# vita-epfl/collaborative-gan-sampling

Hardware: AMD Instinct MI355X
Metric: refined samples/sec @ 20 refinement steps (higher is better)
Workload: dtype f32; 1 GPU; dcgan64 collaborative refinement (propose + K-step refine + render), batch 1024/GPU, K=20, momentum rate 0.1, refine at feature [8, 8, 256], random-init weights, z~U(-1,1) seed 2019+rank; global_batch=1024, refine_steps=20, parallelism=single GPU, hipgraph=True, batches_in_flight=2, fused_per_launch=1, sync_bn=False, contraction=f32

## Files before the change

collaborative-gan-sampling_amd/csrc/api.hip:

```cpp
#include <stdarg.h>
#include <stdio.h>

#include "cgs_internal.h"

static thread_local char g_err[512] = "";
static thread_local const char* g_last_kernel = "";

static thread_local double g_last_flops = 0.0;
static thread_local int g_last_tail[2] = {0, 0};
void cgs_note_tail(int tiles, int split) { g_last_tail[0] = tiles; g_last_tail[1] = split; }
static thread_local int g_contraction = CGS_CONTRACTION_F32;
int cgs_contraction_mode() { return g_contraction; }

void cgs_note_kernel(const char* name) { g_last_kernel = name; }
void cgs_note_flops(double f) { g_last_flops = f; }
void cgs_add_flops(double f) { g_last_flops += f; }

int cgs_set_error(int code, const char* fmt, ...) {
    va_list ap;
    va_start(ap, fmt);
    vsnprintf(g_err, sizeof(g_err), fmt, ap);
    va_end(ap);
    return code;
}

extern "C" {

int cgs_version(void) { return 117; }
const char* cgs_last_error(void) { return g_err; }
const char* cgs_last_kernel(void) { return g_last_kernel; }
double cgs_last_executed_flops(void) { return g_last_flops; }
int cgs_last_tail_tiles(void) { return g_last_tail[0]; }
int cgs_last_tail_split(void) { return g_last_tail[1]; }
int cgs_set_contraction(int mode) {
    if (mode < CGS_CONTRACTION_F32 || mode > CGS_CONTRACTION_BX6_ALL) return cgs_set_error(CGS_EINVAL, "set_contraction: mode %d", mode);
    g_contraction = mode;
    return CGS_OK;
}
int cgs_get_contraction(void) { return g_contraction; }

}

struct ConvCall { CgsLayer L; bool dirT, deconv, bwd; };

static ConvCall conv_call_of(int op, int H, int W, int Cin, int Ho, int Wo, int Cout, int kh, int kw, int sh, int sw) {
    ConvCall c;
    c.deconv = (op == CGS_DECONV_FWD || op == CGS_DECONV_BWD_DATA);
    c.bwd = (op == CGS_CONV_BWD_DATA || op == CGS_DECONV_BWD_DATA);
    c.dirT = (op == CGS_CONV_BWD_DATA || op == CGS_DECONV_FWD);
    CgsLayer& L = c.L;
    L.kh = kh; L.kw = kw; L.sh = sh; L.sw = sw;
    if (!c.deconv) { L.Hb = H; L.Wb = W; L.Cb = Cin; L.Hs = cgs_ceil_div(H, sh > 0 ? sh : 1); L.Ws = cgs_ceil_div(W, sw > 0 ? sw : 1); L.Cs = Cout; }
    else { L.Hs = H; L.Ws = W; L.Cs = Cin; L.Hb = Ho; L.Wb = Wo; L.Cb = Cout; }
    return c;
}

static int check_layer(const CgsLayer& L, const char* who) {
    if (L.kh <= 0 || L.kw <= 0 || L.sh <= 0 || L.sw <= 0 || L.Hb <= 0 || L.Wb <= 0 || L.Cb <= 0 || L.Cs <= 0)
        return cgs_set_error(CGS_EINVAL, "%s: non-positive dimension", who);
    if (L.Hs != cgs_ceil_div(L.Hb, L.sh) || L.Ws != cgs_ceil_div(L.Wb, L.sw))
        return cgs_set_error(CGS_EINVAL, "%s: 'SAME' geometry mismatch: big %dx%d stride %dx%d needs small %dx%d, got %dx%d", who,
// ... 523 lines not shown
```

collaborative-gan-sampling_amd/csrc/bn.hip:

```cpp
#include "cgs_internal.h"

#define BN_MAX_BLOCKS CGS_BN_MAX_BLOCKS

struct BnGeom {
    int G;
    int rows_per_block;
};

static BnGeom bn_geom(int M, int C) {
    BnGeom g;
    int rpb = cgs_ceil_div(M, BN_MAX_BLOCKS);
    if (rpb < 16) rpb = 16;
    g.rows_per_block = rpb;
    g.G = cgs_ceil_div(M, rpb);
    (void)C;
    return g;
}

__device__ __forceinline__ float4 zero4() { return make_float4(0.f, 0.f, 0.f, 0.f); }

__device__ __forceinline__ void bn_affine4(const float* __restrict__ mean, const float* __restrict__ invstd, const float* __restrict__ gamma,
                                           const float* __restrict__ beta, int c, float4& mu, float4& inv, float4& sc, float4& sh) {
    mu = *(const float4*)(mean + c); inv = *(const float4*)(invstd + c);
    const float4 g = *(const float4*)(gamma + c), b = *(const float4*)(beta + c);
// ... 649 lines not shown
        return cgs_set_error(CGS_EWORKSPACE, "groupnorm fwd from partials: workspace %zu < %zu", ws_bytes, (size_t)groups * 4 * C * sizeof(float));
    return norm_fwd_from_partials("groupnorm_lrelu_fwd_from_partials", x, part, groups, rows_per_seg, nseg, seg_stride, gamma, beta, eps, leak, y, mean, invstd,
                                  M_group, C, (float*)ws , nullptr, (hipStream_t)stream);
}

int cgs_norm_lrelu_bwd_from_partials(const float* dy, const float* x, const float* part, int groups, int rows_per_seg, int nseg, int seg_stride,
                                     const float* gamma, const float* beta, const float* mean, const float* invstd, float leak, float* dx,
                                     int M_group, int C, void* ws, size_t ws_bytes, void* stream) {
    const char* who = "norm_lrelu_bwd_from_partials";
    if (groups <= 0 || groups > 65535 || M_group <= 0 || C <= 0 || (C & 3) || rows_per_seg <= 0 || nseg <= 0 || seg_stride < 0 || !part || !dy || !x || !dx)
        return cgs_set_error(CGS_EINVAL, "norm bwd from partials: groups=%d M=%d C=%d rows=%d x %d", groups, M_group, C, rows_per_seg, nseg);
    const bool sliced = groups == 1 && nseg == 1 && rows_per_seg >= 1024 && !((uintptr_t)ws & 7);
    const size_t need = (size_t)groups * 2 * C * sizeof(float) + (sliced ? (size_t)BNF_SLICES * 2 * C * sizeof(double) : 0);
    if (!ws || ws_bytes < need) return cgs_set_error(CGS_EWORKSPACE, "norm bwd from partials: workspace %zu < %zu", ws_bytes, need);
    hipStream_t s = (hipStream_t)stream;
    if (const int rpb = norm_fa_rows_per_block(groups, rows_per_seg, nseg, M_group, C)) {
        hipLaunchKernelGGL(norm_fa_kernel<true>, dim3(cgs_ceil_div(C, 64), cgs_ceil_div(M_group, rpb), groups), dim3(256), 0, s, x, dy, part, rows_per_seg, nseg,
                           seg_stride, gamma, beta, 0.f, leak, dx, (float*)mean, (float*)invstd, M_group, C, rpb);
        return norm_launched(who, "norm_fa_bwd");
    }
    float* stat2 = (float*)ws;
    if (sliced) {
        double* slices = (double*)ws;
        stat2 = (float*)(slices + (size_t)BNF_SLICES * 2 * C);
        hipLaunchKernelGGL(bn_slice_sums_kernel, dim3(cgs_ceil_div(C, BNF_CH), BNF_SLICES), dim3(256), 0, s, part, rows_per_seg, C, slices);
        hipLaunchKernelGGL(bn_finalize2_slices_kernel, dim3(cgs_ceil_div(C, 64)), dim3(64), 0, s, slices, BNF_SLICES, (double)M_group, C, stat2);
    } else {
        hipLaunchKernelGGL(bn_finalize_kernel<1>, dim3(cgs_ceil_div(C, BNF_CH), groups), dim3(256), 0, s, part, rows_per_seg, M_group, C, nullptr, nullptr, 0.f,
                           stat2, nullptr, nullptr, nseg, seg_stride);
    }
    launch_apply_bwd(dy, x, mean, invstd, gamma, beta, stat2, leak, dx, groups, M_group, C, s);
    return norm_launched(who, sliced ? "norm_sliced_bwd" : "norm_finalize_bwd");
}
```

collaborative-gan-sampling_amd/engine.py:

```python
import gc

import numpy as np
import torch

from . import kernels as K
from . import lib as L
from .nets import ARCHS, _same_out, g_input_shape, layer_ks


class _Stage:
    out = None
    bwd_epi = (L.EPI_NONE, None, None)
    pre_folded = False
    bwd_nstat = None
    bstat = None

    def fwd(self, x):
        raise NotImplementedError

    def bwd(self, dy):
        raise NotImplementedError


class _View(_Stage):
# ... 416 lines not shown
            continue
        if isinstance(below, _BnTrainLrelu) and below.sync is None:
            gamma, beta, gimg = below.gamma, below.beta, B // below.groups
        elif isinstance(below, _InstNormAct):
            gamma, beta, gimg = below.scale, below.offset, 1
        else:
            continue
        C = below.out.shape[-1]
        if isinstance(above, _Conv):
            H, W, Cin = above.dx.shape[1:]
            kh, kw, _, Cout = above.w.shape
            lay = K.conv_stat_layout(L.CONV_BWD_DATA, B, H, W, Cin, 0, 0, Cout, kh, kw, above.s, above.s, gimg)
        else:
            lay = K.conv_stat_layout(L.DECONV_BWD_DATA, *above.call_dims(), above.s, above.s, gimg)
        if lay is None:
            continue
        part = torch.empty((lay[0], 2, C), dtype=torch.float32, device=below.out.device)
        below.bstat = above.bwd_nstat = K.NormBwdStats(None, below.mean, below.invstd, gamma, beta, below.leak, gimg, part, lay)
    if stages and isinstance(stages[-1], _Residual):
        link_norm_backward_stats(stages[-1].inner, B)


class Tape:

    def __init__(self, layers, in_shape, P, scope, B, k, stride, bn_training, dev):
        self.folds = []
        self.stages, self.out_shape = compile_layers(layers, in_shape, P, scope, B, k, stride, bn_training, dev, self.folds)

    def forward(self, x):
        for st in self.stages:
            x = st.fwd(x)
        return x

    def backward(self, dy, update=None):
        for st in reversed(self.stages[1:]):
            dy = st.bwd(dy)
        return self.stages[0].bwd(dy) if update is None else self.stages[0].bwd(dy, update=update)


def _entry(fn):
    import functools

    @functools.wraps(fn)
    def wrapped(self, *a, **kw):
        prev = K.set_contraction(self.contraction)
        try:
            return fn(self, *a, **kw)
        finally:
            if prev != self.contraction:
                K.set_contraction(prev)
    return wrapped


class RefineEngine:

    def __init__(self, arch, params, batch_size, device=None, use_graph=False, sync_bn=None, bn_groups=1, contraction="f32"):
        self.A = ARCHS[arch] if isinstance(arch, str) else arch
        if contraction not in L.CONTRACTIONS:
            raise L.CgsError(f"contraction {contraction!r}: expected one of {sorted(L.CONTRACTIONS)}")
        self.contraction = contraction
        self.dev = torch.device(device if device is not None else "cuda:0")
        if self.dev.type != "cuda":
            raise L.CgsError("RefineEngine needs a GPU device (there is no CPU path)")
        L.load()
        prev_mode = K.set_contraction(self.contraction)
        try:
            self._build(params, batch_size, use_graph, sync_bn, bn_groups)
        finally:
# ... 33 lines not shown
                for below, st in zip([None] + stages[:-1], stages):
                    if isinstance(st, _BnTrainLrelu):
                        st.set_groups(self.bn_groups, below if isinstance(below, _Conv) else None)
                    if isinstance(st, _Residual):
                        walk_g(st.inner)
            walk_g(self.d.stages); walk_g(self.g_tail.stages)
        self.sync_bn = None
        if sync_bn is not None and sync_bn is not False:
            if use_graph:
                raise L.CgsError("sync_bn runs eagerly: the all-reduce between the two halves of a bn pass is not captured")
            self.sync_bn = BnSync(None if sync_bn is True else sync_bn)

            def walk(stages):
                for st in stages:
                    if isinstance(st, _BnTrainLrelu):
                        st.sync = self.sync_bn
                    if isinstance(st, _Residual):
                        walk(st.inner)
            walk(self.d.stages); walk(self.g_tail.stages)

        def drop_partials(stages):
            for below, st in zip([None] + stages[:-1], stages):
                if isinstance(st, _BnTrainLrelu) and st.sync is not None:
                    st.part = None
                    if isinstance(below, _Conv):
                        below.part = None
                if isinstance(st, _Residual):
                    drop_partials(st.inner)
        drop_partials(self.d.stages); drop_partials(self.g_tail.stages)
        link_norm_backward_stats(self.g_tail.stages + self.d.stages, B)
        first = self.g_tail.stages[0]
        self.update_form = first.update_form() if isinstance(first, (_Conv, _Deconv)) else None
        self.fused_update = self.update_form is not None and self.update_form[0] != "tail"

    def _sync_weights(self):
        if self._ws_epoch != K.WS.epoch:
            self._resync()

    def _resync(self):
        K.set_contraction(self.contraction)
        epoch = K.WS.epoch
        with torch.cuda.device(self.dev):
            for tape in (self.g_head, self.g_tail, self.d):
                for a, c, gamma, beta, mm, mv in tape.folds:
                    K.bn_fold(gamma, beta, mm, mv, out=(a, c))
            if self._gstream is not None and self._graphs:
                cur = torch.cuda.current_stream(self.dev)
                self._gstream.wait_stream(cur)
                with torch.cuda.stream(self._gstream):
                    self.forward_logits(self.theta, self.logit)
                    self.backward_to_feature()
                cur.wait_stream(self._gstream)
        self._ws_epoch = epoch

    @_entry
    def input_to_feature(self, z):
        self._sync_weights()
        return self.g_head.forward(z)

    @_entry
    def feature_to_data(self, feat):
        self._sync_weights()
        return self.g_tail.forward(feat)

    @_entry
    def discriminator(self, x):
# ... 18 lines not shown
            i -= 1
        st = stages[i] if i >= 0 else None
        active = (isinstance(st, (_Conv, _Linear)) and st.epi != L.EPI_NONE) or (isinstance(st, (_BnTrainLrelu, _InstNormAct)) and st.leak != 1.0) \
            or isinstance(st, _Unary)
        if not active:
            raise L.CgsError("score_with_features: no nonlinearity in front of the discriminator's logit layer")
        return st

    def feature_width(self):
        return int(self._feature_stage().out.shape[-1])

    @_entry
    def score_with_features(self, images, out=None, feat_out=None):
        self._sync_weights()
        st = self._feature_stage()
        sig = K.sigmoid_rowmean(self.d.forward(images), out=out)
        act = st.out
        if act.dim() == 2:
            if feat_out is None:
                return sig, act
            feat_out.copy_(act)
            return sig, feat_out
        if feat_out is None:
            if getattr(self, "_feat", None) is None:
                self._feat = torch.empty((act.shape[0], act.shape[-1]), dtype=torch.float32, device=self.dev)
            feat_out = self._feat
        return sig, K.spatial_mean(act, out=feat_out)

    def forward_logits(self, theta, logit_out, loss="bce", ladam=None, first=False):
        x = self.g_tail.forward(theta)
        head = self.d.stages[-1]
        plain = loss == "bce" and ladam is None
        if isinstance(head, _Linear) and head.w.shape[1] == 1 and head.epi == L.EPI_NONE:
            for st in self.d.stages[:-1]:
                x = st.fwd(x)
            head.x_in = x
            if plain:
                return K.linear_out1_bce(x, head.w, head.b, head.out, self.dlogits, logit_out)
            return K.linear_out1_seed(x, head.w, head.b, head.out, self.dlogits, logit_out, loss, ladam, first)
        logits = self.d.forward(x)
        if plain:
            K.bce_ones_grad_rowmean(logits, self.dlogits, logit_out)
        else:
            K.refine_loss_seed(logits, loss, self.dlogits, logit_out, ladam, first)
        return logits

    def backward_to_feature(self, update=None):
        return self.g_tail.backward(self.d.backward(self.dlogits), update=update)

    @_entry
    def compute_forward_logits_and_grad(self, feature, loss="bce"):
        if loss not in ("bce", "lsq", "linear"):
            raise L.CgsError(f"loss {loss!r}: the engine differentiates 'bce', 'lsq' and 'linear'")
        self._sync_weights()
        self.forward_logits(feature, self.logit, loss)
        return self.logit, self.backward_to_feature()

    def _program(self, steps, rate, alpha, probabilistic, vmin, vmax, loss="bce", ladam=None):
        th = self.theta
        render = self.g_tail.stages[-1].out
        self.forward_logits(th, self.logit, loss, ladam, True)
        self.default_logit.copy_(self.logit)
        self.best_logit.copy_(self.logit)
        self.best_theta.copy_(th)
        self.images.copy_(render)
        self.best_step.fill_(1.0)
        self.tickets.zero_()
        forced = self.forced if probabilistic else None
        fused = self.fused_update and self.update_form is not None and ladam is None and not (vmin and vmax)
        for i in range(steps):
            if fused:
                self.backward_to_feature(update=K.FusedUpdate(th, self.mom, rate, alpha, first=(i == 0)))
                self.forward_logits(th, self.logit, loss, ladam, False)
                K.refine_select2(render, self.images, th, self.best_theta, self.logit, forced, i, self.best_logit, self.best_step, self.tickets)
                continue
            g = self.backward_to_feature()
            if ladam is None:
                K.refine_update(th, self.mom, g, rate, alpha, first=(i == 0), vmin=vmin, vmax=vmax)
            else:
                K.refine_update_ladam(th, self.mom, self.mean_square, g, ladam.gain, rate, first=(i == 0), vmin=vmin, vmax=vmax)
            self.forward_logits(th, self.logit, loss, ladam, False)
            K.refine_select2(render, self.images, th, self.best_theta, self.logit, forced, i, self.best_logit, self.best_step, self.tickets)

    @_entry
    def refine(self, feature0, steps, rate, method="momentum", mode="deterministic", indices=None,
               vmin=None, vmax=None, loss="bce", real_sigmoid_mean=None):
        ladam = None
        if method == "momentum":
            alpha = 0.9
        elif method == "sgd":
            alpha = 0.0
        elif method == "ladam":
            if real_sigmoid_mean is None:
                raise L.CgsError("ladam needs a loss argument the map-space refiner never passes "
                                 "(sampling/collaborator.py:66 vs policy.py:48-51); use momentum or sgd, or pass real_sigmoid_mean")
            alpha = None
        else:
            raise NotImplementedError(method)
        if loss not in ("bce", "lsq", "linear"):
            raise L.CgsError(f"loss {loss!r}: the engine differentiates 'bce', 'lsq' and 'linear'")
        if mode not in ("deterministic", "probabilistic"):
            raise NotImplementedError(mode)
        prob = mode == "probabilistic"
        if prob:
            if indices is None:
                raise L.CgsError("probabilistic mode needs the step indices (np.random.randint(K+1, size=B))")
            self.forced.copy_(torch.as_tensor(np.asarray(indices), dtype=torch.int32))
        if tuple(feature0.shape) != tuple(self.theta.shape):
            raise L.CgsError(f"feature batch {tuple(feature0.shape)} != engine shape {tuple(self.theta.shape)}")
        self._sync_weights()
        with torch.cuda.device(self.dev):
            self.theta.copy_(feature0)
            if method == "ladam":
                if self._ladam is None:
                    self._ladam = K.LadamState(self.B, self.dev)
                    self.mean_square = torch.empty_like(self.mom)
                ladam = self._ladam
                ladam.set_real(real_sigmoid_mean)
            key = (steps, float(rate), alpha, prob, vmin, vmax, loss, method, bool(self.fused_update))
            if not self.use_graph:
                self._program(steps, rate, alpha, prob, vmin, vmax, loss, ladam)
            else:
                g = self._graphs.get(key)
                if g is None:
                    if self._gstream is None:
                        self._gstream = torch.cuda.Stream(self.dev)
                    cur = torch.cuda.current_stream(self.dev)
                    self._gstream.wait_stream(cur)
                    with torch.cuda.stream(self._gstream):
                        self._program(steps, rate, alpha, prob, vmin, vmax, loss, ladam)
                        self.theta.copy_(feature0)
                    torch.cuda.synchronize(self.dev)
                    gc_was_on = gc.isenabled()
                    gc.disable()
                    try:
                        g = torch.cuda.CUDAGraph()
                        with torch.cuda.graph(g, stream=self._gstream, capture_error_mode="thread_local"):
                            self._program(steps, rate, alpha, prob, vmin, vmax, loss, ladam)
                    except L.CgsError:
                        raise
                    except Exception as ex:
                        raise L.GraphCaptureError(f"{type(ex).__name__}: {str(ex)[:300]}") from ex
                    finally:
                        if gc_was_on:
                            gc.enable()
                    cur.wait_stream(self._gstream)
                    self._graphs[key] = g
                g.replay()
        return self.images, self.default_logit, self.best_logit, self.best_step, self.best_theta

    @_entry
    def refresh_weights(self):
# ... 7 lines not shown
```

collaborative-gan-sampling_amd/kernels.py:

```python
import math
import operator
import weakref

import torch

from . import lib as L

LEAK = 0.2
BN_EPS = 1e-5


def _chk(t, name):
    if not (isinstance(t, torch.Tensor) and t.is_cuda and t.dtype == torch.float32 and t.is_contiguous()):
        raise L.CgsError(f"{name}: expected a contiguous fp32 tensor on the GPU, got "
                         f"{type(t).__name__} {getattr(t, 'dtype', None)} {getattr(t, 'device', None)}")
    return t


def _ptr(t):
    return None if t is None else t.data_ptr()


def _stream():
    return torch.cuda.current_stream().cuda_stream
# ... 687 lines not shown
        self.loss_avg = torch.empty(B, dtype=torch.float32, device=device)
        self.gain = torch.empty(B, dtype=torch.float32, device=device)

    def set_real(self, value):
        if isinstance(value, torch.Tensor):
            self.s_real.copy_(value.reshape(1))
        else:
            self.s_real.fill_(float(value))

    def arg(self, first):
        import ctypes
        return ctypes.byref(L.LadamSeed(_ptr(self.s_real), _ptr(self.loss_avg), _ptr(self.gain), 1 if first else 0))


def refine_loss_seed(logits, kind, dlogits=None, logit_mean=None, ladam=None, first=False):
    _chk(logits, "logits")
    B = logits.shape[0]
    dl = dlogits if dlogits is not None else torch.empty_like(logits)
    lm = logit_mean if logit_mean is not None else torch.empty(B, dtype=torch.float32, device=logits.device)
    L.call("cgs_refine_loss_seed", _ptr(logits), _loss_kind(kind, ("bce", "lsq", "linear")), _ptr(dl), _ptr(lm), B, logits.numel() // B,
           None if ladam is None else ladam.arg(first), _stream())
    return dl, lm


def linear_out1_seed(x, w, bias, logits, dlogits, logit_mean, kind, ladam=None, first=False):
    _chk(x, "x"); _chk(w, "w")
    B, K = x.shape
    pr = _Prof(2.0 * B * K, "", _nb(x, w, logits), op="linear_out1_fwd") if PROFILE is not None else None
    L.call("cgs_linear_out1_seed", _ptr(x), _ptr(w), _ptr(bias), _ptr(logits), _ptr(dlogits), _ptr(logit_mean), B, K,
           _loss_kind(kind, ("bce", "lsq", "linear")), None if ladam is None else ladam.arg(first), _stream())
    if pr is not None:
        pr.done()
    return logits


def ladam_gain(loss, loss_avg, gain, first):
    for t, name in ((loss, "loss"), (loss_avg, "loss_avg"), (gain, "gain")):
        _chk(t, name)
    B = loss.numel()
    if loss_avg.numel() != B or gain.numel() != B:
        raise L.CgsError("ladam_gain: loss, loss_avg and gain must have one size")
    L.call("cgs_ladam_gain", _ptr(loss), _ptr(loss_avg), _ptr(gain), 1 if first else 0, B, _stream())
    return gain


def refine_update_ladam(theta, m, v, g, gain, rate, first, vmin=None, vmax=None):
    for t, name in ((theta, "theta"), (m, "m"), (v, "v"), (g, "g"), (gain, "gain")):
        _chk(t, name)
    B = theta.shape[0]
    if m.numel() != theta.numel() or v.numel() != theta.numel() or g.numel() != theta.numel() or gain.numel() < B:
        raise L.CgsError("refine_update_ladam: theta, m, v and g must have one size, gain at least B elements")
    use_clip = 1 if (vmin and vmax) else 0
    pr = _Prof(0.0, "", _nb(theta, theta, m, v, g) + (0.0 if first else _nb(m, v)), op="refine_update_ladam") if PROFILE is not None else None
    L.call("cgs_refine_update_ladam", _ptr(theta), _ptr(m), _ptr(v), _ptr(g), _ptr(gain), float(rate), 1 if first else 0, use_clip,
           float(vmin or 0.0), float(vmax or 0.0), B, theta.numel() // B, _stream())
    if pr is not None:
        pr.done()


def refine_select_rows(src, logit, forced, step_index, dst, best_logit):
    B = src.shape[0]
    L.call("cgs_refine_select_rows", _ptr(src), _ptr(logit), _ptr(forced), step_index, _ptr(dst), _ptr(best_logit),
           B, src.numel() // B, _stream())


_wgrad_ws = {}
# ... 513 lines not shown
```

collaborative-gan-sampling_amd/lib.py:

```python
import ctypes as C
import os

_HERE = os.path.dirname(os.path.abspath(__file__))
LIB_PATH = os.environ.get("CGS_LIB") or os.path.join(_HERE, "libcgs_hip.so")

OK, EINVAL, EWORKSPACE, ELAUNCH = 0, -1, -2, -3
EPI_NONE, EPI_LRELU, EPI_AFFINE_RELU, EPI_TANH = 0, 1, 2, 3
EPI_RELU_BWD_AFFINE, EPI_LRELU_BWD, EPI_TANH_BWD = 4, 5, 6
CONV_FWD, CONV_BWD_DATA, DECONV_FWD, DECONV_BWD_DATA = 0, 1, 2, 3
FAMILY_IGEMM, FAMILY_QUAD, FAMILY_SMALLN_T, FAMILY_SMALLN_F, FAMILY_PATCH, FAMILY_TAPS, FAMILY_DOT, FAMILY_IGEMM_BX6 = 0, 1, 2, 3, 4, 5, 6, 7
CONTRACTION_F32, CONTRACTION_BX6, CONTRACTION_BX6_ALL = 0, 1, 2
CONTRACTIONS = {"f32": CONTRACTION_F32, "bx6": CONTRACTION_BX6, "bx6_all": CONTRACTION_BX6_ALL}
LOSS_BCE, LOSS_LSQ, LOSS_LINEAR, LOSS_HINGE = 0, 1, 2, 3
LOSSES = {"bce": LOSS_BCE, "lsq": LOSS_LSQ, "linear": LOSS_LINEAR, "hinge": LOSS_HINGE}


class LadamSeed(C.Structure):
    _fields_ = [("s_real", C.c_void_p), ("loss_avg", C.c_void_p), ("gain", C.c_void_p), ("first", C.c_int)]


_p, _i, _f, _z = C.c_void_p, C.c_int, C.c_float, C.c_size_t
_ll = C.c_longlong

SIGNATURES = {
# ... 10 lines not shown
    "cgs_conv_ws_bytes_for": (_z, [_i] * 10),
    "cgs_conv_family": (_i, [_i] * 13 + [_z]),
    "cgs_conv2d_nhwc_fwd": (_i, [_p] * 4 + [_i] * 9 + [_i, _p, _p, _p, _z, _i, _p]),
    "cgs_conv_stat_partials": (_i, [_i] * 9 + [_z]),
    "cgs_conv2d_nhwc_fwd_stats": (_i, [_p] * 4 + [_i] * 9 + [_p, _z, _i, _p, _z, _p]),
    "cgs_conv_stat_layout": (_i, [_i] * 13 + [_z, _p, _p, _p]),
    "cgs_deconv2d_nhwc_fwd_stats": (_i, [_p] * 4 + [_i] * 11 + [_p, _z, _i, _p, _z, _p]),
    "cgs_conv2d_nhwc_bwd_data_nstats": (_i, [_p] * 3 + [_i] * 9 + [_p] * 5 + [_f, _i, _p, _z, _i, _p, _z, _p]),
    "cgs_deconv2d_nhwc_bwd_data_nstats": (_i, [_p] * 3 + [_i] * 11 + [_p] * 5 + [_f, _i, _p, _z, _i, _p, _z, _p]),
    "cgs_norm_lrelu_bwd_from_partials": (_i, [_p] * 3 + [_i] * 4 + [_p] * 4 + [_f, _p, _i, _i, _p, _z, _p]),
    "cgs_groupnorm_lrelu_fwd_from_partials": (_i, [_p, _p, _i, _i, _i, _i, _p, _p, _f, _f, _p, _p, _p, _i, _i, _p, _z, _p]),
    "cgs_bn_train_lrelu_fwd_from_partials": (_i, [_p, _p, _i, _p, _p, _f, _f, _p, _p, _p, _i, _i, _p, _z, _p]),
    "cgs_conv2d_nhwc_bwd_data": (_i, [_p] * 3 + [_i] * 9 + [_i, _p, _p, _p, _z, _i, _p]),
    "cgs_deconv2d_nhwc_fwd": (_i, [_p] * 4 + [_i] * 11 + [_i, _p, _p, _p, _z, _i, _p]),
    "cgs_deconv2d_nhwc_bwd_data": (_i, [_p] * 3 + [_i] * 11 + [_i, _p, _p, _p, _z, _i, _p]),
    "cgs_conv_update_form": (_i, [_i] * 12 + [_z, _p]),
    "cgs_conv2d_nhwc_bwd_data_update": (_i, [_p] * 4 + [_i] * 9 + [_f, _f, _i, _p, _z, _i, _p]),
    "cgs_deconv2d_nhwc_bwd_data_update": (_i, [_p] * 4 + [_i] * 11 + [_f, _f, _i, _p, _z, _i, _p]),
    "cgs_conv_signs_ok": (_i, [_i] * 13 + [_z]),
    "cgs_deconv2d_nhwc_fwd_signs": (_i, [_p] * 4 + [_i] * 11 + [_i, _p, _p, _p, _p, _z, _i, _p]),
    "cgs_deconv2d_nhwc_bwd_data_signs": (_i, [_p] * 3 + [_i] * 11 + [_i, _p, _p, _p, _z, _i, _p]),
    "cgs_linear_fwd": (_i, [_p] * 4 + [_i] * 4 + [_p, _z, _i, _p]),
    "cgs_linear_bwd_data": (_i, [_p] * 3 + [_i] * 3 + [_p, _z, _i, _p]),
    "cgs_bn_ws_bytes": (_z, [_i, _i]),
    "cgs_bn_train_lrelu_fwd": (_i, [_p, _p, _p, _f, _f, _p, _p, _p, _i, _i, _p, _z, _p]),
    "cgs_bn_train_lrelu_bwd_data": (_i, [_p] * 6 + [_f, _p, _i, _i, _p, _z, _p]),
    "cgs_bn_sync_fwd_sums": (_i, [_p, _p, _i, _i, _p, _z, _p]),
    "cgs_bn_sync_fwd_apply": (_i, [_p, _p, _p, _f, _f, _p, _ll, _p, _p, _p, _i, _i, _p, _z, _p]),
    "cgs_bn_sync_bwd_sums": (_i, [_p] * 6 + [_f, _p, _i, _i, _p, _z, _p]),
    "cgs_bn_sync_bwd_apply": (_i, [_p] * 6 + [_f, _p, _ll, _p, _i, _i, _p, _z, _p]),
    "cgs_instnorm_ws_bytes": (_z, [_i, _i, _i]),
    "cgs_instnorm_lrelu_fwd": (_i, [_p, _p, _p, _f, _f, _p, _p, _p, _i, _i, _i, _p, _z, _p]),
    "cgs_instnorm_lrelu_bwd_data": (_i, [_p] * 6 + [_f, _p, _i, _i, _i, _p, _z, _p]),
    "cgs_add": (_i, [_p, _p, _p, _z, _p]),
    "cgs_bn_fold": (_i, [_p] * 4 + [_f, _p, _p, _i, _p]),
    "cgs_affine_relu_fwd": (_i, [_p] * 4 + [_i, _i, _p]),
    "cgs_affine_relu_bwd": (_i, [_p] * 4 + [_i, _i, _p]),
    "cgs_affine_fwd": (_i, [_p] * 4 + [_i, _i, _p]),
    "cgs_affine_bwd": (_i, [_p] * 3 + [_i, _i, _p]),
    "cgs_lrelu_fwd": (_i, [_p, _f, _p, _z, _p]),
    "cgs_lrelu_bwd": (_i, [_p, _p, _f, _p, _z, _p]),
    "cgs_tanh_fwd": (_i, [_p, _p, _z, _p]),
    "cgs_tanh_bwd": (_i, [_p, _p, _p, _z, _p]),
    "cgs_bce_ones_grad_rowmean": (_i, [_p, _p, _p, _i, _i, _p]),
    "cgs_bce_ones_fwd": (_i, [_p, _p, _z, _p]),
    "cgs_bce_ones_bwd": (_i, [_p, _p, _p, _z, _p]),
    "cgs_sigmoid_rowmean": (_i, [_p, _p, _i, _i, _p]),
    "cgs_clip": (_i, [_p, _f, _f, _p, _z, _p]),
    "cgs_refine_update": (_i, [_p, _p, _p, _f, _f, _i, _i, _f, _f, _z, _p]),
    "cgs_refine_select": (_i, [_p, _p, _p, _i, _p, _p, _p, _i, _i, _p]),
    "cgs_refine_select_rows": (_i, [_p, _p, _p, _i, _p, _p, _i, _i, _p]),
    "cgs_refine_select2": (_i, [_p, _p, _i, _p, _p, _i, _p, _p, _i, _p, _p, _p, _i, _p]),
    "cgs_linear_out1_bce": (_i, [_p, _p, _p, _p, _p, _p, _i, _i, _p]),
    "cgs_linear_out1_seed": (_i, [_p, _p, _p, _p, _p, _p, _i, _i, _i, _p, _p]),
    "cgs_refine_loss_seed": (_i, [_p, _i, _p, _p, _i, _i, _p, _p]),
    "cgs_refine_update_ladam": (_i, [_p, _p, _p, _p, _p, _f, _i, _i, _f, _f, _i, _i, _p]),
    "cgs_ladam_gain": (_i, [_p, _p, _p, _i, _i, _p]),
    "cgs_gan_logits_grad": (_i, [_p, _i, _f, _f, _p, _p, _i, _p]),
    "cgs_gan_loss": (_i, [_p, _i, _f, _p, _p, _z, _p]),
    "cgs_mlp2d_sigmoid_saliency": (_i, [_p, _p, _i, _i, _p, _p, _p, _i, _f, _p]),
    "cgs_refine2d": (_i, [_p, _p, _i, _i, _p, _f, _f, _i, _f, _i, _p, _p, _p, _i, _p]),
    "cgs_refine2d_devbase": (_i, [_p, _p, _i, _i, _p, _p, _f, _i, _f, _i, _p, _p, _p, _i, _p]),
    "cgs_mlp2d_train_ws_bytes": (_z, [_i, _i]),
    "cgs_mlp2d_d_step": (_i, [_p, _p, _i, _i, _p, _i, _p, _i, _f, _p, _p, _p, _p, _z, _p]),
    "cgs_mlp2d_wide_train_ws_bytes": (_z, [_i, _i, _i]),
    "cgs_mlp2d_wide_d_step": (_i, [_p, _p, _i, _i, _p, _i, _p, _i, _f, _p, _p, _p, _p, _z, _p]),
# ... 145 lines not shown
```

include/cgs_hip.h:

```cpp
#ifndef CGS_HIP_H
#define CGS_HIP_H

#include <stddef.h>
#include <stdint.h>

#ifdef __cplusplus
extern "C" {
#endif

#define CGS_OK 0
#define CGS_EINVAL (-1)
#define CGS_EWORKSPACE (-2)
#define CGS_ELAUNCH (-3)

#define CGS_EPI_NONE 0
#define CGS_EPI_LRELU 1
#define CGS_EPI_AFFINE_RELU 2
#define CGS_EPI_TANH 3
#define CGS_EPI_RELU_BWD_AFFINE 4
#define CGS_EPI_LRELU_BWD 5
#define CGS_EPI_TANH_BWD 6

#define CGS_CONV_FWD 0
#define CGS_CONV_BWD_DATA 1
// ... 121 lines not shown
int cgs_linear_bwd_data(const float* dy, const float* w, float* dx, int B, int in, int out,
                        void* ws, size_t ws_bytes, int ws_prepacked, void* stream);

size_t cgs_bn_ws_bytes(int M, int C);
int cgs_bn_train_lrelu_fwd(const float* x, const float* gamma, const float* beta, float eps, float leak,
                           float* y, float* mean, float* invstd, int M, int C,
                           void* ws, size_t ws_bytes, void* stream);
int cgs_bn_train_lrelu_fwd_from_partials(const float* x, const float* part, int G, const float* gamma, const float* beta,
                                         float eps, float leak, float* y, float* mean, float* invstd, int M, int C,
                                         void* ws, size_t ws_bytes, void* stream);
int cgs_bn_train_lrelu_bwd_data(const float* dy, const float* x, const float* gamma, const float* beta,
                                const float* mean, const float* invstd, float leak, float* dx, int M, int C,
                                void* ws, size_t ws_bytes, void* stream);

int cgs_bn_sync_fwd_sums(const float* x, double* sums, int M, int C, void* ws, size_t ws_bytes, void* stream);
int cgs_bn_sync_fwd_apply(const float* x, const float* gamma, const float* beta, float eps, float leak, const double* sums,
                          long long M_total, float* y, float* mean, float* invstd, int M, int C,
                          void* ws, size_t ws_bytes, void* stream);
int cgs_bn_sync_bwd_sums(const float* dy, const float* x, const float* gamma, const float* beta, const float* mean,
                         const float* invstd, float leak, double* sums, int M, int C, void* ws, size_t ws_bytes, void* stream);
int cgs_bn_sync_bwd_apply(const float* dy, const float* x, const float* gamma, const float* beta, const float* mean,
                          const float* invstd, float leak, const double* sums, long long M_total, float* dx, int M, int C,
                          void* ws, size_t ws_bytes, void* stream);

size_t cgs_instnorm_ws_bytes(int B, int HW, int C);
int cgs_instnorm_lrelu_fwd(const float* x, const float* scale, const float* offset, float eps, float leak, float* y,
                           float* mean, float* invstd, int B, int HW, int C, void* ws, size_t ws_bytes, void* stream);
int cgs_instnorm_lrelu_bwd_data(const float* dy, const float* x, const float* scale, const float* offset,
                                const float* mean, const float* invstd, float leak, float* dx, int B, int HW, int C,
                                void* ws, size_t ws_bytes, void* stream);
int cgs_groupnorm_lrelu_fwd_from_partials(const float* x, const float* part, int groups, int rows_per_seg, int nseg, int seg_stride,
                                          const float* gamma, const float* beta, float eps, float leak, float* y, float* mean,
                                          float* invstd, int M_group, int C, void* ws, size_t ws_bytes, void* stream);
int cgs_add(const float* a, const float* b, float* out, size_t n, void* stream);

int cgs_bn_fold(const float* gamma, const float* beta, const float* moving_mean, const float* moving_var,
                float eps, float* a, float* b, int C, void* stream);
int cgs_affine_relu_fwd(const float* x, const float* a, const float* b, float* y, int M, int C, void* stream);
int cgs_affine_relu_bwd(const float* dy, const float* y, const float* a, float* dx, int M, int C, void* stream);
int cgs_affine_fwd(const float* x, const float* a, const float* b, float* y, int M, int C, void* stream);
int cgs_affine_bwd(const float* dy, const float* a, float* dx, int M, int C, void* stream);
int cgs_lrelu_fwd(const float* x, float leak, float* y, size_t n, void* stream);
int cgs_lrelu_bwd(const float* dy, const float* y, float leak, float* dx, size_t n, void* stream);
int cgs_tanh_fwd(const float* x, float* y, size_t n, void* stream);
int cgs_tanh_bwd(const float* dy, const float* y, float* dx, size_t n, void* stream);

int cgs_bce_ones_grad_rowmean(const float* logits, float* dlogits, float* logit_mean, int B, int P, void* stream);
int cgs_refine_loss_seed(const float* logits, int kind, float* dlogits, float* logit_mean, int B, int P, const cgs_ladam_seed* ladam,
                         void* stream);

int cgs_bce_ones_fwd(const float* logits, float* loss, size_t n, void* stream);
int cgs_bce_ones_bwd(const float* dloss, const float* logits, float* dlogits, size_t n, void* stream);
int cgs_sigmoid_rowmean(const float* logits, float* sigmoids, int B, int P, void* stream);
int cgs_gan_loss(const float* logits, int kind, float target, const float* dloss, float* out, size_t n, void* stream);
int cgs_clip(const float* x, float vmin, float vmax, float* y, size_t n, void* stream);

int cgs_refine_update(float* theta, float* m, const float* g, float rate, float alpha, int first,
                      int use_clip, float vmin, float vmax, size_t n, void* stream);
int cgs_ladam_gain(const float* loss, float* loss_avg, float* gain, int first, int B, void* stream);
int cgs_refine_update_ladam(float* theta, float* m, float* v, const float* g, const float* gain, float rate, int first, int use_clip,
                            float vmin, float vmax, int B, int F, void* stream);
int cgs_refine_select(const float* theta, const float* logit, const int32_t* forced, int step_index,
                      float* best_theta, float* best_logit, float* best_step, int B, int F, void* stream);
int cgs_refine_select2(const float* rows, float* best_rows, int Frows, const float* theta, float* best_theta, int F, const float* logit,
                       const int32_t* forced, int step_index, float* best_logit, float* best_step, int* tickets, int B, void* stream);
int cgs_refine_select_rows(const float* src, const float* logit, const int32_t* forced, int step_index, float* dst,
// ... 114 lines not shown
```

Measured before the change: 6711 samples/s.

## Fuse final batchnorm+lrelu with linear head in discriminator forward and backward

Adds kernels that compute the last BN+LeakyReLU on the fly inside the 1-output linear head's dot product. This avoids writing the normalized activation and then re-reading it for a separate GEMV. The backward pass rebuilds dy as dlogits times w inside the BN backward sums and apply kernels, which skips materializing the head gradient and the separate head backward. The path is used only for batch norm with one group and no sync BN, and it is disabled on the single-step gradient API. In exchange the backward reads the activation input twice, adds new reduction kernels, and adds a fused_head flag to the graph cache key.

```diff
diff --git a/collaborative-gan-sampling_amd/csrc/api.hip b/collaborative-gan-sampling_amd/csrc/api.hip
--- a/collaborative-gan-sampling_amd/csrc/api.hip
+++ b/collaborative-gan-sampling_amd/csrc/api.hip
@@ -26,7 +26,7 @@
 
 extern "C" {
 
-int cgs_version(void) { return 117; }
+int cgs_version(void) { return 118; }
 const char* cgs_last_error(void) { return g_err; }
 const char* cgs_last_kernel(void) { return g_last_kernel; }
 double cgs_last_executed_flops(void) { return g_last_flops; }
diff --git a/collaborative-gan-sampling_amd/csrc/bn.hip b/collaborative-gan-sampling_amd/csrc/bn.hip
--- a/collaborative-gan-sampling_amd/csrc/bn.hip
+++ b/collaborative-gan-sampling_amd/csrc/bn.hip
@@ -705,3 +705,189 @@
     launch_apply_bwd(dy, x, mean, invstd, gamma, beta, stat2, leak, dx, groups, M_group, C, s);
     return norm_launched(who, sliced ? "norm_sliced_bwd" : "norm_finalize_bwd");
 }
+
+template <int KIND, bool LADAM>
+__global__ __launch_bounds__(256) void norm_head_fwd_kernel(const float* __restrict__ y, const float* __restrict__ stat0 ,
+                                                            float leak, const float* __restrict__ w, const float* __restrict__ bias,
+                                                            float* __restrict__ logits, float* __restrict__ dl, float* __restrict__ lm, int B,
+                                                            int K, int C, int samples_per_group, cgs_ladam_seed la) {
+    const int b = blockIdx.x * 4 + (threadIdx.x >> 6);
+    const int lane = threadIdx.x & 63;
+    if (b >= B) return;
+    const float* row = y + (size_t)b * K;
+    const float* stat = stat0 + (size_t)(b / samples_per_group) * 4 * C;
+    const int cstep = 256 % C;
+    int c = (lane * 4) % C;
+    float s = 0.f;
+#pragma unroll 4
+    for (int k = lane * 4; k < K; k += 256) {
+        float4 sc, sh;
+        apply_fwd_params(stat, C, c, sc, sh);
+        const float4 a = norm_fwd4(*(const float4*)(row + k), sc, sh, leak), ww = *(const float4*)(w + k);
+        s = fmaf(a.x, ww.x, s); s = fmaf(a.y, ww.y, s); s = fmaf(a.z, ww.z, s); s = fmaf(a.w, ww.w, s);
+        c += cstep;
+        if (c >= C) c -= C;
+    }
+#pragma unroll
+    for (int off = 32; off > 0; off >>= 1) s += __shfl_down(s, off, 64);
+    if (lane == 0) {
+        const float v = s + (bias ? bias[0] : 0.f);
+        logits[b] = v;
+        dl[b] = loss_seed1<KIND>(v);
+        lm[b] = v;
+        if (LADAM) ladam_seed1(la, b, sigmoid_stable(v));
+    }
+}
+
+__device__ __forceinline__ float4 head_dy4(const float* __restrict__ dl, const float* __restrict__ w, int R, int HW, int C, int cq) {
+    const int b = R / HW, p = R - b * HW;
+    const float g = dl[b];
+    const float4 wv = ((const float4*)(w + (size_t)p * C))[cq];
+    return make_float4(g * wv.x, g * wv.y, g * wv.z, g * wv.w);
+}
+
+__global__ __launch_bounds__(256) void norm_head_bwd_sums_kernel(const float* __restrict__ x, const float* __restrict__ dl, const float* __restrict__ w,
+                                                                 const float* __restrict__ mean_p, const float* __restrict__ invstd_p,
+                                                                 const float* __restrict__ gamma, const float* __restrict__ beta, float leak,
+                                                                 float* __restrict__ part, int M, int C, int HW, int rows_per_block) {
+    __shared__ float4 red[2][256];
+    const int R0 = blockIdx.y * M;
+    x += (size_t)R0 * C; mean_p += (size_t)blockIdx.y * C; invstd_p += (size_t)blockIdx.y * C;
+    part += (size_t)blockIdx.y * gridDim.x * 2 * C;
+    const int tid = threadIdx.x;
+    const int r0 = blockIdx.x * rows_per_block;
+    const int r1 = min(M, r0 + rows_per_block);
+    const int CQ = C >> 2;
+    int tpr = 1;
+    while (tpr * 2 <= CQ && tpr * 2 <= 256) tpr *= 2;
+    const int rg = tid / tpr, RG = 256 / tpr, tc = tid - rg * tpr;
+    for (int q0 = 0; q0 < CQ; q0 += tpr) {
+        const int cq = q0 + tc;
+        float4 sa = zero4(), sb = sa;
+        if (cq < CQ) {
+            float4 mean, invstd, scale, shift;
+            bn_affine4(mean_p, invstd_p, gamma, beta, 4 * cq, mean, invstd, scale, shift);
+            for (int r = r0 + rg; r < r1; r += RG) {
+                const float4 xv = ((const float4*)(x + (size_t)r * C))[cq];
+                norm_d_acc4(xv, head_dy4(dl, w, R0 + r, HW, C, cq), mean, invstd, scale, shift, leak, sa, sb);
+            }
+        }
+        red[0][tid] = sa; red[1][tid] = sb;
+        __syncthreads();
+        if (rg == 0 && cq < CQ) {
+            float4 ta = zero4(), tb = ta;
+            for (int gq = 0; gq < RG; ++gq) {
+                const float4 a = red[0][gq * tpr + tc], b = red[1][gq * tpr + tc];
+                add4(ta, a); add4(tb, b);
+            }
+            ((float4*)(part + ((size_t)blockIdx.x * 2 + 0) * C))[cq] = ta;
+            ((float4*)(part + ((size_t)blockIdx.x * 2 + 1) * C))[cq] = tb;
+        }
+        __syncthreads();
+    }
+}
+
+__global__ __launch_bounds__(256) void norm_head_bwd_apply_kernel(const float* __restrict__ x, const float* __restrict__ dl, const float* __restrict__ w,
+                                                                  const float* __restrict__ mean0, const float* __restrict__ invstd0,
+                                                                  const float* __restrict__ gamma, const float* __restrict__ beta,
+                                                                  const float* __restrict__ stat20, float leak, float* __restrict__ dx, int B, int K,
+                                                                  int C, int samples_per_group) {
+    const int k = (blockIdx.x * 256 + threadIdx.x) * 4;
+    if (k >= K) return;
+    const int c = k % C;
+    const float4 wv = *(const float4*)(w + k);
+    float4 mean, inv, sc, sh, m1, m2;
+    int grp = -1;
+    for (int b = blockIdx.y; b < B; b += gridDim.y) {
+        if (b / samples_per_group != grp) {
+            grp = b / samples_per_group;
+            apply_bwd_params(mean0, invstd0, gamma, beta, stat20, grp, C, c, mean, inv, sc, sh, m1, m2);
+        }
+        const float g = dl[b];
+        const float4 dy = make_float4(g * wv.x, g * wv.y, g * wv.z, g * wv.w);
+        const size_t i = (size_t)b * K + k;
+        *(float4*)(dx + i) = norm_bwd4(*(const float4*)(x + i), dy, mean, inv, sc, sh, m1, m2, leak);
+    }
+}
+
+int cgs_norm_head_form(int norm, int groups, int sync, int head_out, int B, int K, int C) {
+    if (norm != 0 || sync || head_out != 1) return 0;
+    if (B <= 0 || K <= 0 || C <= 0 || groups <= 0 || groups > 65535) return 0;
+    if ((K & 3) || (C & 3) || K % C || B % groups) return 0;
+    if ((long long)B * K > 0x7fffffffLL) return 0;
+    return 1;
+}
+
+struct HeadGeom { int HW, M; BnGeom g; NormWs w; };
+static HeadGeom head_geom(int B, int K, int C, int groups, void* ws) {
+    HeadGeom h;
+    h.HW = K / C; h.M = B / groups * h.HW;
+    h.g = groups == 1 ? bn_geom(h.M, C) : in_geom(groups, h.M);
+    h.w = groups == 1 ? bn_ws(ws, C) : carve_ws(ws, groups, C, cgs_instnorm_stat2_offset(groups, h.M, C));
+    return h;
+}
+static size_t head_ws_bytes(int B, int K, int C, int groups) {
+    const int M = B / groups * (K / C);
+    return groups == 1 ? cgs_bn_ws_bytes(M, C) : cgs_instnorm_ws_bytes(groups, M, C);
+}
+
+int cgs_norm_head_fwd(const float* y, const float* part, int groups, int rows_per_seg, int nseg, int seg_stride, const float* gamma,
+                      const float* beta, float eps, float leak, float* mean, float* invstd, const float* w, const float* bias, float* logits,
+                      float* dlogits, float* logit_mean, int B, int K, int C, int kind, const cgs_ladam_seed* ladam, void* ws, size_t ws_bytes,
+                      void* stream) {
+    const char* who = "norm_head_fwd";
+    if (!cgs_norm_head_form(0, groups, 0, 1, B, K, C)) return cgs_set_error(CGS_EINVAL, "%s: not offered for B=%d K=%d C=%d groups=%d (cgs_norm_head_form)", who, B, K, C, groups);
+    if (!y || !part || !gamma || !beta || !mean || !invstd || !w || !logits || !dlogits || !logit_mean || rows_per_seg <= 0 || nseg <= 0 || seg_stride < 0)
+        return cgs_set_error(CGS_EINVAL, "%s: bad argument", who);
+    if (kind != CGS_LOSS_BCE && kind != CGS_LOSS_LSQ && kind != CGS_LOSS_LINEAR) return cgs_set_error(CGS_EINVAL, "%s: kind %d", who, kind);
+    if (ladam && (!ladam->s_real || !ladam->loss_avg || !ladam->gain)) return cgs_set_error(CGS_EINVAL, "%s: ladam state with a null pointer", who);
+    const size_t need = groups == 1 ? cgs_bn_ws_bytes(B * (K / C), C) : (size_t)groups * 4 * C * sizeof(float);
+    if (!ws || ws_bytes < need) return cgs_set_error(CGS_EWORKSPACE, "%s: workspace %zu < %zu", who, ws_bytes, need);
+    hipStream_t s = (hipStream_t)stream;
+    const int M = B / groups * (K / C);
+    float* stat = groups == 1 ? bn_ws(ws, C).stat : (float*)ws;
+    if (groups == 1 && nseg == 1 && rows_per_seg >= 1024 && !((uintptr_t)ws & 7)) {
+        double* slices = (double*)ws;
+        hipLaunchKernelGGL(bn_slice_sums_kernel, dim3(cgs_ceil_div(C, BNF_CH), BNF_SLICES), dim3(256), 0, s, part, rows_per_seg, C, slices);
+        hipLaunchKernelGGL(bn_finalize_slices_kernel, dim3(cgs_ceil_div(C, 64)), dim3(64), 0, s, slices, BNF_SLICES, (double)M, C, gamma, beta, eps, stat, mean, invstd);
+    } else {
+        hipLaunchKernelGGL(bn_finalize_kernel<0>, dim3(cgs_ceil_div(C, BNF_CH), groups), dim3(256), 0, s, part, rows_per_seg, M, C, gamma, beta, eps, stat,
+                           mean, invstd, nseg, seg_stride);
+    }
+    const dim3 grid(cgs_ceil_div(B, 4)), block(256);
+    const cgs_ladam_seed la = ladam ? *ladam : cgs_ladam_seed{};
+    const int spg = B / groups;
+#define HEAD_FWD(KIND, LADAM) hipLaunchKernelGGL((norm_head_fwd_kernel<KIND, LADAM>), grid, block, 0, s, y, stat, leak, w, bias, logits, dlogits, logit_mean, B, K, C, spg, la)
+    if (kind == CGS_LOSS_BCE) { if (ladam) HEAD_FWD(CGS_LOSS_BCE, true); else HEAD_FWD(CGS_LOSS_BCE, false); }
+    else if (kind == CGS_LOSS_LSQ) { if (ladam) HEAD_FWD(CGS_LOSS_LSQ, true); else HEAD_FWD(CGS_LOSS_LSQ, false); }
+    else { if (ladam) HEAD_FWD(CGS_LOSS_LINEAR, true); else HEAD_FWD(CGS_LOSS_LINEAR, false); }
+#undef HEAD_FWD
+    return norm_launched(who, "norm_head_fwd");
+}
+
+int cgs_norm_head_bwd_sums(const float* y, const float* dlogits, const float* w, const float* gamma, const float* beta, const float* mean,
+                           const float* invstd, float leak, int B, int K, int C, int groups, void* ws, size_t ws_bytes, void* stream) {
+    const char* who = "norm_head_bwd_sums";
+    if (!cgs_norm_head_form(0, groups, 0, 1, B, K, C)) return cgs_set_error(CGS_EINVAL, "%s: not offered for B=%d K=%d C=%d groups=%d (cgs_norm_head_form)", who, B, K, C, groups);
+    if (!y || !dlogits || !w || !gamma || !beta || !mean || !invstd) return cgs_set_error(CGS_EINVAL, "%s: bad argument", who);
+    if (!ws || ws_bytes < head_ws_bytes(B, K, C, groups)) return cgs_set_error(CGS_EWORKSPACE, "%s: workspace %zu < %zu", who, ws_bytes, head_ws_bytes(B, K, C, groups));
+    const HeadGeom h = head_geom(B, K, C, groups, ws);
+    hipLaunchKernelGGL(norm_head_bwd_sums_kernel, dim3(h.g.G, groups), dim3(256), 0, (hipStream_t)stream, y, dlogits, w, mean, invstd, gamma, beta, leak, h.w.part,
+                       h.M, C, h.HW, h.g.rows_per_block);
+    return norm_launched(who, "norm_head_bwd_sums");
+}
+
+int cgs_norm_head_bwd_apply(const float* y, const float* dlogits, const float* w, const float* gamma, const float* beta, const float* mean,
+                            const float* invstd, float leak, float* dx, int B, int K, int C, int groups, void* ws, size_t ws_bytes, void* stream) {
+    const char* who = "norm_head_bwd_apply";
+    if (!cgs_norm_head_form(0, groups, 0, 1, B, K, C)) return cgs_set_error(CGS_EINVAL, "%s: not offered for B=%d K=%d C=%d groups=%d (cgs_norm_head_form)", who, B, K, C, groups);
+    if (!y || !dlogits || !w || !gamma || !beta || !mean || !invstd || !dx) return cgs_set_error(CGS_EINVAL, "%s: bad argument", who);
+    if (!ws || ws_bytes < head_ws_bytes(B, K, C, groups)) return cgs_set_error(CGS_EWORKSPACE, "%s: workspace %zu < %zu", who, ws_bytes, head_ws_bytes(B, K, C, groups));
+    const HeadGeom h = head_geom(B, K, C, groups, ws);
+    hipStream_t s = (hipStream_t)stream;
+    hipLaunchKernelGGL(bn_finalize_kernel<1>, dim3(cgs_ceil_div(C, BNF_CH), groups), dim3(256), 0, s, h.w.part, h.g.G, h.M, C, nullptr, nullptr, 0.f, h.w.stat2, nullptr,
+                       nullptr);
+    hipLaunchKernelGGL(norm_head_bwd_apply_kernel, dim3(cgs_ceil_div(K, 1024), B < 65535 ? B : 65535), dim3(256), 0, s, y, dlogits, w, mean, invstd, gamma, beta,
+                       h.w.stat2, leak, dx, B, K, C, B / groups);
+    return norm_launched(who, "norm_head_bwd_apply");
+}
diff --git a/collaborative-gan-sampling_amd/engine.py b/collaborative-gan-sampling_amd/engine.py
--- a/collaborative-gan-sampling_amd/engine.py
+++ b/collaborative-gan-sampling_amd/engine.py
@@ -472,8 +472,8 @@
             x = st.fwd(x)
         return x
 
-    def backward(self, dy, update=None):
-        for st in reversed(self.stages[1:]):
+    def backward(self, dy, update=None, top=None):
+        for st in reversed(self.stages[1:top]):
             dy = st.bwd(dy)
         return self.stages[0].bwd(dy) if update is None else self.stages[0].bwd(dy, update=update)
 
@@ -573,6 +573,26 @@
         first = self.g_tail.stages[0]
         self.update_form = first.update_form() if isinstance(first, (_Conv, _Deconv)) else None
         self.fused_update = self.update_form is not None and self.update_form[0] != "tail"
+        self.head_plan = self._plan_fused_head()
+        self.fused_head = self.head_plan is not None and self.head_plan[1].groups == 1
+
+    def _plan_fused_head(self):
+        stages = self.d.stages
+        head = stages[-1]
+        if not (isinstance(head, _Linear) and head.w.shape[1] == 1 and head.epi == L.EPI_NONE):
+            return None
+        i = len(stages) - 2
+        while i >= 0 and isinstance(stages[i], _View):
+            i -= 1
+        st = stages[i] if i >= 0 else None
+        if not isinstance(st, _BnTrainLrelu) or st.part is None or st.bstat is not None:
+            return None
+        if st.groups > 1 and st.part_layout is None:
+            return None
+        Kin, C = head.w.shape[0], st.out.shape[-1]
+        if st.out.numel() != self.B * Kin:
+            return None
+        return (i, st) if K.norm_head_form(st.groups, st.sync is not None, 1, self.B, Kin, C) else None
 
     def _sync_weights(self):
         if self._ws_epoch != K.WS.epoch:
@@ -657,6 +677,13 @@
         head = self.d.stages[-1]
         plain = loss == "bce" and ladam is None
         if isinstance(head, _Linear) and head.w.shape[1] == 1 and head.epi == L.EPI_NONE:
+            if self.fused_head and self.head_plan is not None:
+                top, norm = self.head_plan
+                for st in self.d.stages[:top]:
+                    x = st.fwd(x)
+                norm.x = x
+                return K.norm_head_fwd(x, norm.part, norm.part_layout if norm.groups > 1 else None, norm.groups, norm.gamma, norm.beta, norm.leak,
+                                       (norm.mean, norm.invstd), head.w, head.b, head.out, self.dlogits, logit_out, loss, ladam, first)
             for st in self.d.stages[:-1]:
                 x = st.fwd(x)
             head.x_in = x
@@ -671,6 +698,13 @@
         return logits
 
     def backward_to_feature(self, update=None):
+        if self.fused_head and self.head_plan is not None:
+            top, norm = self.head_plan
+            head = self.d.stages[-1]
+            a = (norm.x, self.dlogits, head.w, norm.gamma, norm.beta, norm.mean, norm.invstd, norm.leak, norm.groups)
+            K.norm_head_bwd_sums(*a)
+            dy = K.norm_head_bwd_apply(*a, out=norm.out)
+            return self.g_tail.backward(self.d.backward(dy, top=top), update=update)
         return self.g_tail.backward(self.d.backward(self.dlogits), update=update)
 
     @_entry
@@ -678,8 +712,12 @@
         if loss not in ("bce", "lsq", "linear"):
             raise L.CgsError(f"loss {loss!r}: the engine differentiates 'bce', 'lsq' and 'linear'")
         self._sync_weights()
-        self.forward_logits(feature, self.logit, loss)
-        return self.logit, self.backward_to_feature()
+        keep, self.fused_head = self.fused_head, False
+        try:
+            self.forward_logits(feature, self.logit, loss)
+            return self.logit, self.backward_to_feature()
+        finally:
+            self.fused_head = keep
 
     def _program(self, steps, rate, alpha, probabilistic, vmin, vmax, loss="bce", ladam=None):
         th = self.theta
@@ -742,7 +780,7 @@
                     self.mean_square = torch.empty_like(self.mom)
                 ladam = self._ladam
                 ladam.set_real(real_sigmoid_mean)
-            key = (steps, float(rate), alpha, prob, vmin, vmax, loss, method, bool(self.fused_update))
+            key = (steps, float(rate), alpha, prob, vmin, vmax, loss, method, bool(self.fused_update), bool(self.fused_head))
             if not self.use_graph:
                 self._program(steps, rate, alpha, prob, vmin, vmax, loss, ladam)
             else:
diff --git a/collaborative-gan-sampling_amd/kernels.py b/collaborative-gan-sampling_amd/kernels.py
--- a/collaborative-gan-sampling_amd/kernels.py
+++ b/collaborative-gan-sampling_amd/kernels.py
@@ -743,6 +743,58 @@
     if pr is not None:
         pr.done()
     return logits
+
+
+def norm_head_form(groups, sync, head_out, B, K, C, norm="batch"):
+    return bool(L.load().cgs_norm_head_form(0 if norm == "batch" else 1, int(groups), 1 if sync else 0, int(head_out), int(B), int(K), int(C)))
+
+
+def _norm_head_ws(B, K, C, groups, device):
+    M = B // groups * (K // C)
+    return _in_workspace(groups, M, C, device) if groups > 1 else _bn_workspace(M, C, device)
+
+
+def norm_head_fwd(y, part, layout, groups, gamma, beta, leak, stats, w, bias, logits, dlogits, logit_mean, kind="bce", ladam=None, first=False,
+                  eps=BN_EPS):
+    _chk(y, "y"); _chk(part, "part"); _chk(w, "w")
+    B, C_ = y.shape[0], y.shape[-1]
+    K = y.numel() // B
+    lay = layout if layout is not None else (part.shape[0], part.shape[0], 1, 0)
+    ws = _norm_head_ws(B, K, C_, groups, y.device)
+    pr = _Prof(0.0, "", _nb(y, w, logits), op="norm_head_fwd") if PROFILE is not None else None
+    L.call("cgs_norm_head_fwd", _ptr(y), _ptr(part), groups, lay[1], lay[2], lay[3], _ptr(gamma), _ptr(beta), eps, leak, _ptr(stats[0]),
+           _ptr(stats[1]), _ptr(w), _ptr(bias), _ptr(logits), _ptr(dlogits), _ptr(logit_mean), B, K, C_,
+           _loss_kind(kind, ("bce", "lsq", "linear")), None if ladam is None else ladam.arg(first), _ptr(ws), ws.numel() * 4, _stream())
+    if pr is not None:
+        pr.done()
+    return logits
+
+
+def norm_head_bwd_sums(y, dlogits, w, gamma, beta, mean, invstd, leak, groups=1):
+    _chk(y, "y"); _chk(w, "w")
+    B, C_ = y.shape[0], y.shape[-1]
+    K = y.numel() // B
+    ws = _norm_head_ws(B, K, C_, groups, y.device)
+    pr = _Prof(0.0, "", _nb(y, w), op="norm_head_bwd_sums") if PROFILE is not None else None
+    L.call("cgs_norm_head_bwd_sums", _ptr(y), _ptr(dlogits), _ptr(w), _ptr(gamma), _ptr(beta), _ptr(mean), _ptr(invstd), leak, B, K, C_, groups,
+           _ptr(ws), ws.numel() * 4, _stream())
+    if pr is not None:
+        pr.done()
+    return ws
+
+
+def norm_head_bwd_apply(y, dlogits, w, gamma, beta, mean, invstd, leak, groups=1, out=None):
+    _chk(y, "y"); _chk(w, "w")
+    B, C_ = y.shape[0], y.shape[-1]
+    K = y.numel() // B
+    dx = out if out is not None else torch.empty_like(y)
+    ws = _norm_head_ws(B, K, C_, groups, y.device)
+    pr = _Prof(0.0, "", _nb(y, w, dx), op="norm_head_bwd_apply") if PROFILE is not None else None
+    L.call("cgs_norm_head_bwd_apply", _ptr(y), _ptr(dlogits), _ptr(w), _ptr(gamma), _ptr(beta), _ptr(mean), _ptr(invstd), leak, _ptr(dx), B, K, C_,
+           groups, _ptr(ws), ws.numel() * 4, _stream())
+    if pr is not None:
+        pr.done()
+    return dx
 
 
 def ladam_gain(loss, loss_avg, gain, first):
diff --git a/collaborative-gan-sampling_amd/lib.py b/collaborative-gan-sampling_amd/lib.py
--- a/collaborative-gan-sampling_amd/lib.py
+++ b/collaborative-gan-sampling_amd/lib.py
@@ -66,6 +66,10 @@
     "cgs_instnorm_ws_bytes": (_z, [_i, _i, _i]),
     "cgs_instnorm_lrelu_fwd": (_i, [_p, _p, _p, _f, _f, _p, _p, _p, _i, _i, _i, _p, _z, _p]),
     "cgs_instnorm_lrelu_bwd_data": (_i, [_p] * 6 + [_f, _p, _i, _i, _i, _p, _z, _p]),
+    "cgs_norm_head_form": (_i, [_i] * 7),
+    "cgs_norm_head_fwd": (_i, [_p, _p, _i, _i, _i, _i, _p, _p, _f, _f, _p, _p, _p, _p, _p, _p, _p, _i, _i, _i, _i, _p, _p, _z, _p]),
+    "cgs_norm_head_bwd_sums": (_i, [_p] * 7 + [_f, _i, _i, _i, _i, _p, _z, _p]),
+    "cgs_norm_head_bwd_apply": (_i, [_p] * 7 + [_f, _p, _i, _i, _i, _i, _p, _z, _p]),
     "cgs_add": (_i, [_p, _p, _p, _z, _p]),
     "cgs_bn_fold": (_i, [_p] * 4 + [_f, _p, _p, _i, _p]),
     "cgs_affine_relu_fwd": (_i, [_p] * 4 + [_i, _i, _p]),
diff --git a/include/cgs_hip.h b/include/cgs_hip.h
--- a/include/cgs_hip.h
+++ b/include/cgs_hip.h
@@ -177,6 +177,18 @@
 int cgs_groupnorm_lrelu_fwd_from_partials(const float* x, const float* part, int groups, int rows_per_seg, int nseg, int seg_stride,
                                           const float* gamma, const float* beta, float eps, float leak, float* y, float* mean,
                                           float* invstd, int M_group, int C, void* ws, size_t ws_bytes, void* stream);
+
+int cgs_norm_head_form(int norm, int groups, int sync, int head_out, int B, int K, int C);
+int cgs_norm_head_fwd(const float* y, const float* part, int groups, int rows_per_seg, int nseg, int seg_stride, const float* gamma,
+                      const float* beta, float eps, float leak, float* mean, float* invstd, const float* w, const float* bias,
+                      float* logits, float* dlogits, float* logit_mean, int B, int K, int C, int kind, const cgs_ladam_seed* ladam,
+                      void* ws, size_t ws_bytes, void* stream);
+int cgs_norm_head_bwd_sums(const float* y, const float* dlogits, const float* w, const float* gamma, const float* beta,
+                           const float* mean, const float* invstd, float leak, int B, int K, int C, int groups,
+                           void* ws, size_t ws_bytes, void* stream);
+int cgs_norm_head_bwd_apply(const float* y, const float* dlogits, const float* w, const float* gamma, const float* beta,
+                            const float* mean, const float* invstd, float leak, float* dx, int B, int K, int C, int groups,
+                            void* ws, size_t ws_bytes, void* stream);
 int cgs_add(const float* a, const float* b, float* out, size_t n, void* stream);
 
 int cgs_bn_fold(const float* gamma, const float* beta, const float* moving_mean, const float* moving_var,
```

After: 6723 samples/s (median of 3 runs). Within noise of the previous version (+0.2%).
